# xubiker/deephisto

Hardware: AMD Instinct MI355X
Metric: 256x256 patches/sec WSI inference (predict_full_patched) (higher is better)
Workload: dtype bf16

## Files before the change

### deephisto_amd/_lib.py

```python
from __future__ import annotations

import ctypes as C
from pathlib import Path

import torch

LIB_PATH = Path(__file__).resolve().parent / "libdeephisto_hip.so"

DH_LAYOUT_NHWC, DH_LAYOUT_NCHW = 0, 1
DH_DTYPE_F32, DH_DTYPE_BF16 = 0, 1

_i32, _i64, _u32 = C.c_int32, C.c_int64, C.c_uint32
BUCKET_CB = C.CFUNCTYPE(None, C.c_int32, C.c_int64, C.c_int64, C.c_void_p)
_p = C.c_void_p

SIGNATURES = {
    "dh_abi_version": (C.c_int, []),
    "dh_last_error": (C.c_char_p, []),
    "dh_tile_grid_count": (C.c_int, [_i64, _i64, _i32, _i32, _i32, C.POINTER(_i64), C.POINTER(_i64)]),
    "dh_tile_grid": (C.c_int, [_i64, _i64, _i32, _i32, _i32, _p, _i64]),
    "dh_synth_slide": (C.c_int, [_p, _i64, _i64, _u32, _p]),
    "dh_tile_gather": (C.c_int, [_p, _i64, _i64, _p, _p, _i64, _i32, _i32, _i32, _p, _p]),
    "dh_tile_gather_aug": (C.c_int, [_p, _i64, _i64, _p, _i64, _i32, _i32, _i32, _i32, _i32, _p, _p]),
    "dh_tile_gather_raw": (C.c_int, [_p, _i64, _i64, _p, _i64, _i32, _p, _p]),
# ... 24 lines not shown
    "dh_resnet18_bucket": (C.c_int, [_p, _i32, C.POINTER(_i64), C.POINTER(_i64)]),
    "dh_train2_create": (C.c_int, [C.POINTER(_p), C.c_char_p, _i32]),
    "dh_train2_destroy": (None, [_p]),
    "dh_train2_tensor": (C.c_int, [_p, C.c_char_p, _i32, _p, _i64, _i32, _p]),
    "dh_train2_flat": (C.c_int, [_p, _i32, C.POINTER(_p), C.POINTER(_i64)]),
    "dh_train2_set_buckets": (C.c_int, [_p, _i64, _p, _p, C.POINTER(_i32)]),
    "dh_train2_bucket": (C.c_int, [_p, _i32, C.POINTER(_i64), C.POINTER(_i64)]),
    "dh_train2_forward": (C.c_int, [_p, _p, _i64, _i32, _p, _i32, _p]),
    "dh_train2_backward": (C.c_int, [_p, _p, _p]),
    "dh_train2_adam_step": (C.c_int, [_p, C.c_float, C.c_float, C.c_float, C.c_float, _i64, _p]),
    "dh_grad_pack_bf16": (C.c_int, [_p, _p, _i64, _p]),
    "dh_grad_unpack_bf16": (C.c_int, [_p, _p, _i64, C.c_float, _p]),
    "dh_train2_backward_adam": (C.c_int, [_p, _p, C.c_float, C.c_float, C.c_float, C.c_float, _i64, _p]),
    "dh_profile_start": (C.c_int, [_i32, _i32]),
    "dh_profile_stop": (C.c_int, [C.POINTER(C.c_double), C.POINTER(C.c_double), C.POINTER(_i64)]),
}


DEBUG_SIGNATURES = {
    "dh_train2_debug_act": (C.c_int, [_p, C.c_char_p, _i32, _p, _i64, _p]),
    "dh_debug_gemm1x1_bf16": (C.c_int, [_p, _p, _p, _p, _i64] + [_i32] * 8 + [_p]),
    "dh_debug_gemm1x1_fused_bf16": (C.c_int, [_p] * 7 + [_i64] + [_i32] * 8 + [_p]),
    "dh_debug_gemm1x1_bwdsums_bf16": (C.c_int, [_p] * 10 + [_i32, _p, _i64, _i32, _i32, _p]),
    "dh_debug_bn2_bf16": (C.c_int, [_p, _p, _p, _p, _i32, _p, _p, _p, _p, _i32, _p, _p, _p, _p, _i64, _i32, _p]),
    "dh_debug_stem_wgrad_bf16": (C.c_int, [_p, _p, _p, _i32, _i32, _p]),
    "dh_debug_bn2_pool_bf16": (C.c_int, [_p, _p, _p, _p, _p, _p, _p, _p, _p, _p, _p, _i32, _i32, _i32, _i32, _p]),
    "dh_debug_maxpool2_bf16": (C.c_int, [_p, _p, _p, _p, _i32, _i32, _i32, _i32, _p]),
    "dh_debug_upsample2_add_bf16": (C.c_int, [_p, _p] + [_i32] * 6 + [_p]),
    "dh_debug_avgpool_fc_dgrad2": (C.c_int, [_p, _p, _p] + [_i32] * 4 + [_p]),
    "dh_debug_wgrad_bf16": (C.c_int, [_p, _p, _p] + [_i32] * 8 + [_p]),
    "dh_debug_conv_bn_act": (C.c_int, [_p, _p, _p, _p, _p, _p] + [_i32] * 9 + [_p]),
    "dh_debug_stem_out": (C.c_int, [_p, _i64, _i32, _p, _p]),
    "dh_debug_stem_pool_bf16": (C.c_int, [_p, _p, _i64, _i64, _p, _i64, _i32, _p, _p]),
    "dh_debug_wgrad_f32": (C.c_int, [_p, _p, _p] + [_i32] * 8 + [_p]),
    "dh_debug_stem_wgrad_f32": (C.c_int, [_p, _p, _p, _i32, _i32, _p]),
    "dh_debug_dgrad_f32": (C.c_int, [_p, _p, _p, _p] + [_i32] * 7 + [_p]),
    "dh_debug_pack_f32": (C.c_int, [_p, _i32, _i32, _p, _p, _p, _p, _p]),
    "dh_debug_pack_bf16": (C.c_int, [_p, _i32, _i32, _p, _p, _p, _p, _p]),
    "dh_debug_bn_f32": (C.c_int, [_p, _p, _p, _p, _i32, _p, _p, _p, _p, _p, _p, _p, _i64, _i32, _p]),
    "dh_debug_maxpool_f32": (C.c_int, [_p, _p, _p, _p, _i32, _i32, _i32, _i32, _p]),
    "dh_debug_bn_pool_f32": (C.c_int, [_p, _p, _p, _p, _p, _p, _p, _p, _p, _i32, _i32, _i32, _i32, _p]),
    "dh_debug_stamps": (C.c_int, [_i32, _p]),
    "dh_debug_env_knobs": (C.c_int, [C.c_char_p, _i64]),
}


class DeephistoHipError(RuntimeError):
    pass


_lib = None


def lib() -> C.CDLL:
    global _lib
    if _lib is None:
        if not LIB_PATH.exists():
            raise DeephistoHipError(
                f"{LIB_PATH} is missing: build it with `python -m deephisto_amd.build` "
                "(hipcc --offload-arch=gfx950). There is no CPU fallback for the HIP path.")
        h = C.CDLL(str(LIB_PATH))
        for name, (res, args) in {**SIGNATURES, **DEBUG_SIGNATURES}.items():
            fn = getattr(h, name)
            fn.restype, fn.argtypes = res, args
        _lib = h
    return _lib
# ... 7 lines not shown
```

### deephisto_amd/csrc/resnet_kernels.hip

```cpp
#include <math.h>
#include <stdlib.h>
#include <string.h>

#include <algorithm>
#include <array>
#include <map>
#include <mutex>
#include <set>
#include <string>
#include <vector>

#include "dh_common.h"
#include "conv3_tables_host.h"

typedef float f32x16 __attribute__((ext_vector_type(16)));
typedef __bf16 bf16x8 __attribute__((ext_vector_type(8)));

namespace {

constexpr int CHUNK_BYTES = 64;
constexpr int PIX_PITCH = 80;
constexpr int FRAG_BYTES = 1024;
constexpr int SLAB_TAP = 4 * FRAG_BYTES;

// ... 532 lines not shown
            }
}

void pack_stem_weights(const float* w, int esz, std::vector<uint8_t>& out) {
  auto slot = [&](int co, int kh, int i) -> float {
    if (i < 1 || i > 21) return 0.f;
    const int kw = (i - 1) / 3, c = (i - 1) % 3;
    return w[((size_t)(co * 3 + c) * 7 + kh) * 7 + kw];
  };
  if (esz == 2) {
    out.assign((size_t)7 * 2 * 2 * FRAG_BYTES, 0);
    size_t o = 0;
    for (int kh = 0; kh < 7; ++kh)
      for (int t = 0; t < 2; ++t)
        for (int mt = 0; mt < 2; ++mt)
          for (int l = 0; l < 64; ++l)
            for (int j = 0; j < 8; ++j) {
              const uint16_t hb = host_bf16(slot(mt * 32 + (l & 31), kh, 16 * t + 8 * (l >> 5) + j));
              memcpy(&out[o], &hb, 2); o += 2;
            }
  } else {
    out.assign((size_t)7 * 11 * 2 * 256, 0);
    size_t o = 0;
    for (int kh = 0; kh < 7; ++kh)
      for (int s = 0; s < 11; ++s)
        for (int mt = 0; mt < 2; ++mt)
          for (int l = 0; l < 64; ++l) {
            const float v = slot(mt * 32 + (l & 31), kh, 2 * s + (l >> 5));
            memcpy(&out[o], &v, 4); o += 4;
          }
  }
}

void pack_stem_pool_weights(const float* w, std::vector<uint8_t>& out) {
  out.assign((size_t)SP_WBYTES, 0);
  size_t o = 0;
  for (int ks = 0; ks < SP_KS; ++ks)
    for (int mt = 0; mt < 2; ++mt)
      for (int l = 0; l < 64; ++l)
        for (int j = 0; j < 8; ++j) {
          int kh, sl;
          sp_kslot(ks, l >> 5, j, &kh, &sl);
          float v = 0.f;
          if (kh >= 0 && sl >= 1 && sl <= 21) {
            const int co = mt * 32 + (l & 31), kw = (sl - 1) / 3, c = (sl - 1) % 3;
            v = w[((size_t)(co * 3 + c) * 7 + kh) * 7 + kw];
          }
          const uint16_t hb = host_bf16(v);
          memcpy(&out[o], &hb, 2); o += 2;
        }
}

bool g_stamps_on = false;
unsigned long long* g_stamps_dev = nullptr;

struct Profiler {
  bool on = false;
  int every = 1, counter = 0;
  std::vector<hipEvent_t> ev;
  size_t used = 0;
  double flops = 0.0;
} g_prof;

std::mutex g_host_mu;
inline int current_device() { int d = 0; (void)hipGetDevice(&d); return d; }

int ensure_dyn_lds(const void* fn, int bytes) {
  static std::set<std::pair<const void*, int>> done;
  const std::pair<const void*, int> key(fn, current_device());
  std::lock_guard<std::mutex> lk(g_host_mu);
  if (done.count(key)) return DH_OK;
  DH_HIP(hipFuncSetAttribute(fn, hipFuncAttributeMaxDynamicSharedMemorySize, bytes));
  done.insert(key);
  return DH_OK;
}

template <typename T, int KS, int STRIDE, bool HALO>
int launch_conv(const ConvParams& p, hipStream_t st) {
  const int npx_lds = HALO ? p.IMGS * (p.TH + 2) * (p.TW + 2) : 256;
  const size_t lds = (size_t)KS * KS * SLAB_TAP + (size_t)npx_lds * PIX_PITCH;
  const int blocks_per_img = p.tiles_y * p.tiles_x;
  const int groups = ((p.B + p.IMGS - 1) / p.IMGS) * blocks_per_img;
  const int grid = groups * (p.Cout / 64);
// ... 517 lines not shown
  if (net->fc_w_dev) (void)hipFree(net->fc_w_dev);
  if (net->fc_b_dev) (void)hipFree(net->fc_b_dev);
  if (net->ws) (void)hipFree(net->ws);
  delete net;
}

extern "C" int dh_resnet18_set_param(dh_resnet18* net, const char* name, const float* data,
                                     int64_t n_elem) {
  DH_REQUIRE(net && name && data, "resnet18 set_param: null argument");
  const int64_t want = expected_elems(net, name);
  DH_REQUIRE(want >= 0, "resnet18 set_param: unknown parameter '%s'", name);
  DH_REQUIRE(want == n_elem, "resnet18 set_param: '%s' has %lld elements, expected %lld", name,
             (long long)n_elem, (long long)want);
  net->params[name].assign(data, data + n_elem);
  net->finalized = false;
  return DH_OK;
}

extern "C" int dh_resnet18_finalize(dh_resnet18* net, void* stream) {
  DH_REQUIRE(net != nullptr, "resnet18 finalize: null handle");
  (void)stream;
  auto get = [&](const std::string& k) -> const std::vector<float>* {
    auto it = net->params.find(k);
    return it == net->params.end() ? nullptr : &it->second;
  };
  const int esz = net->esz();
  for (size_t i = 0; i < net->convs.size(); ++i) {
    ConvLayer& c = net->convs[i];
    const auto* w = get(c.name + ".weight");
    const auto *g = get(c.bn + ".weight"), *b = get(c.bn + ".bias"), *m = get(c.bn + ".running_mean"),
               *v = get(c.bn + ".running_var");
    DH_REQUIRE(w && g && b && m && v, "resnet18 finalize: parameters of '%s' / '%s' are not all set",
               c.name.c_str(), c.bn.c_str());
    std::vector<uint8_t> packed;
    if (i == 0 && esz == 2) pack_stem_pool_weights(w->data(), packed);
    else if (i == 0) pack_stem_weights(w->data(), esz, packed);
    else pack_conv_weights(w->data(), c.cout, c.cin, c.ks, esz, packed);
    int rc = upload(packed, &c.w_dev);
    if (rc) return rc;
    const bool wide3 = esz == 2 && c.ks == 3 && c.stride == 2 && c.cout % 128 == 0 && c.cin % 16 == 0;
    const bool wide1 = esz == 2 && c.ks == 1 && c.stride == 2 && c.cout % 128 == 0 && c.cin % 16 == 0;
    if (wide3 || wide1) {
      std::vector<uint8_t> packed2;
      pack_conv_weights_wide(w->data(), c.cout, c.cin, c.ks, packed2);
      if ((rc = upload(packed2, &c.w2_dev))) return rc;
    }
    std::vector<float> sc(c.cout), sh(c.cout);
    for (int k = 0; k < c.cout; ++k) {
      const double s = (double)(*g)[k] / sqrt((double)(*v)[k] + 1e-5);
      sc[k] = (float)s;
      sh[k] = (float)((double)(*b)[k] - (double)(*m)[k] * s);
    }
    rc = upload(sc, reinterpret_cast<void**>(&c.scale_dev));
    if (rc) return rc;
    rc = upload(sh, reinterpret_cast<void**>(&c.shift_dev));
    if (rc) return rc;
  }
  const auto *fw = get("fc.weight"), *fb = get("fc.bias");
  DH_REQUIRE(fw && fb, "resnet18 finalize: fc.weight / fc.bias are not set");
  int rc = upload(*fw, reinterpret_cast<void**>(&net->fc_w_dev));
  if (rc) return rc;
  rc = upload(*fb, reinterpret_cast<void**>(&net->fc_b_dev));
  if (rc) return rc;
  net->finalized = true;
  return DH_OK;
}

static int check_forward_args(dh_resnet18* net, int64_t n, int32_t P, const void* logits) {
  DH_REQUIRE(net && (logits || n == 0), "resnet18 forward: null argument");
  DH_REQUIRE(net->finalized, "resnet18 forward: call dh_resnet18_finalize after setting parameters");
  DH_REQUIRE(n >= 0 && n <= 4096, "resnet18 forward: batch %lld out of range [0, 4096]", (long long)n);
  DH_REQUIRE(P >= 32 && P <= 1024, "resnet18 forward: patch %d out of range [32, 1024]", P);
  return DH_OK;
}

extern "C" int dh_resnet18_forward(dh_resnet18* net, const float* x, int64_t n, int32_t P,
                                   float* logits, void* stream) {
  int rc = check_forward_args(net, n, P, logits);
  if (rc) return rc;
  if (n == 0) return DH_OK;
  DH_REQUIRE(x != nullptr, "resnet18 forward: null input");
  hipStream_t st = dh::as_stream(stream);
  return net->dtype == DH_DTYPE_F32
             ? forward_impl<float>(net, x, nullptr, 0, 0, nullptr, n, P, logits, st)
// ... 68 lines not shown
  DH_LAUNCH_CHECK();
  return DH_OK;
}

namespace {
__global__ void blocked_to_nhwc_f32_kernel(const __bf16* in, float* out, int64_t n, int hw) {
  const int64_t total = n * hw * 64;
  for (int64_t i = blockIdx.x * (int64_t)blockDim.x + threadIdx.x; i < total; i += (int64_t)gridDim.x * blockDim.x) {
    const int c = (int)(i % 64);
    const int64_t px = (i / 64) % hw, b = i / 64 / hw;
    out[i] = (float)in[((b * 2 + c / 32) * hw + px) * 32 + c % 32];
  }
}
}

extern "C" int dh_debug_stem_pool_bf16(dh_resnet18* net, const uint8_t* slide_dev, int64_t slide_h, int64_t slide_w,
                                       const int32_t* yx_dev, int64_t n, int32_t P, float* out_dev, void* stream) {
  DH_REQUIRE(net && net->finalized && net->dtype == DH_DTYPE_BF16, "debug stem pool: needs a finalized bf16 network");
  DH_REQUIRE(slide_dev && yx_dev && out_dev && n > 0 && n <= (1 << 20) && P >= 32 && P <= 1024, "debug stem pool: bad arguments");
  hipStream_t st = dh::as_stream(stream);
  const int H1 = (P + 6 - 7) / 2 + 1, H2 = (H1 + 2 - 3) / 2 + 1;
  void* tmp = nullptr;
  DH_HIP(hipMalloc(&tmp, (size_t)n * H2 * H2 * 64 * 2));
  int rc = launch_stem_pool(net, nullptr, slide_dev, slide_h, slide_w, yx_dev, (int)n, P, tmp, st);
  if (!rc) {
    hipLaunchKernelGGL(blocked_to_nhwc_f32_kernel, dim3(1024), dim3(256), 0, st, static_cast<const __bf16*>(tmp), out_dev, n, H2 * H2);
    if (hipGetLastError() != hipSuccess) rc = DH_EHIP;
    (void)hipStreamSynchronize(st);
  }
  (void)hipFree(tmp);
  return rc;
}

extern "C" int dh_profile_start(int32_t sample_every, int32_t max_samples) {
  DH_REQUIRE(sample_every > 0 && max_samples > 0 && max_samples <= (1 << 20), "profile start: bad arguments");
  for (hipEvent_t e : g_prof.ev) (void)hipEventDestroy(e);
  g_prof.ev.assign((size_t)max_samples * 2, nullptr);
  for (auto& e : g_prof.ev) DH_HIP(hipEventCreate(&e));
  g_prof.every = sample_every; g_prof.counter = 0; g_prof.used = 0; g_prof.flops = 0.0;
  g_prof.on = true;
  return DH_OK;
}

extern "C" int dh_profile_stop(double* total_ms, double* total_flops, int64_t* n_samples) {
  g_prof.on = false;
  double ms = 0.0;
  for (size_t i = 0; i + 1 < g_prof.used; i += 2) {
    DH_HIP(hipEventSynchronize(g_prof.ev[i + 1]));
    float t = 0.f;
    DH_HIP(hipEventElapsedTime(&t, g_prof.ev[i], g_prof.ev[i + 1]));
    ms += t;
  }
  if (total_ms) *total_ms = ms;
  if (total_flops) *total_flops = g_prof.flops;
  if (n_samples) *n_samples = (int64_t)(g_prof.used / 2);
  for (hipEvent_t e : g_prof.ev) (void)hipEventDestroy(e);
  g_prof.ev.clear(); g_prof.used = 0;
  return DH_OK;
}

extern "C" int dh_debug_stamps(int32_t enable, unsigned long long* out64_host) {
  g_stamps_on = enable != 0;
  if (out64_host) {
    if (!g_stamps_dev) { memset(out64_host, 0, 64 * sizeof(unsigned long long)); return DH_OK; }
    DH_HIP(hipDeviceSynchronize());
    DH_HIP(hipMemcpy(out64_host, g_stamps_dev, 64 * sizeof(unsigned long long), hipMemcpyDeviceToHost));
// ... 13 lines not shown
```

### deephisto_amd/csrc/stem_pool.inc

```
#ifndef SP_ABL
#define SP_ABL 0
#endif
constexpr int SP_W = 4;
constexpr int SP_T = SP_W * 64;
constexpr int SP_CR = 2 * SP_W, SP_CC = 32;
constexpr int SP_PR = SP_W, SP_PC = 15;
constexpr int SP_WR = 2 * SP_CR + 5;
constexpr int SP_WE = 224;
#ifndef SP_PF
#define SP_PF 3
#endif
constexpr int SP_KS = 11;
constexpr int SP_WBYTES = SP_KS * 2 * FRAG_BYTES;
constexpr int SP_WINB = ((SP_WR * SP_WE * 2 + 255) / 256) * 256;
constexpr int SP_XCH = 4096;
constexpr int SP_LDS = SP_WBYTES + SP_WINB + (SP_W + 1) * SP_XCH + 512;
constexpr int SP_DW = 52;
constexpr int SP_NLOAD = (SP_WR * SP_DW + SP_T - 1) / SP_T;
static_assert(3 * ((SP_LDS + 511) / 512 * 512) <= 160 * 1024, "three workgroups per CU");

inline void sp_kslot(int ks, int hh, int j, int* kh, int* s) {
  *kh = -1; *s = 0;
  if (ks < 9) {
    const int pz = ks / 3, u = ks % 3;
    if (u == 0) { *kh = 2 * pz; *s = 8 * hh + j; }
    else if (u == 1) { *kh = 2 * pz + hh; *s = hh ? j : 16 + j; }
    else { *kh = 2 * pz + 1; *s = 8 + 8 * hh + j; }
  } else if (ks == 9) { *kh = 6; *s = 8 * hh + j; }
  else if (hh == 0) { *kh = 6; *s = 16 + j; }
}

struct StemPoolParams {
  const float* x_nchw; const uint8_t* slide; const int32_t* yx; int64_t row_bytes, slide_bytes;
  const void* w; const float* scale; const float* shift; void* out;
  int B, P, Hc, Wc, Hp, Wp, tiles_y, tiles_x, nstrips, iters;
  unsigned long long* stamps;
};

typedef unsigned short sp_u16x2 __attribute__((ext_vector_type(2)));

template <bool SRC_U8, bool STAMP>
__global__ __launch_bounds__(SP_T, 3) void stem_pool_kernel(const StemPoolParams p) {
  extern __shared__ __attribute__((aligned(16))) char smem[];
  char* w_lds = smem;
  char* win_lds = smem + SP_WBYTES;
  char* xch_lds = win_lds + SP_WINB;
  float* ss_lds = reinterpret_cast<float*>(xch_lds + (SP_W + 1) * SP_XCH);
  const int tid = threadIdx.x, lane = tid & 63, tx = lane & 31, h = lane >> 5;
  const int wave = __builtin_amdgcn_readfirstlane(tid >> 6);
  for (int i = wave; i < SP_WBYTES / 1024; i += SP_W)
    lds_dma<16>(static_cast<const char*>(p.w) + i * 1024 + lane * 16, __builtin_amdgcn_readfirstlane(lds_addr_of(w_lds + i * 1024)));
  if (tid < 128) ss_lds[tid] = tid < 64 ? p.scale[tid] : p.shift[tid - 64];
  for (int i = tid * 16; i < SP_WINB; i += SP_T * 16) *reinterpret_cast<uint4*>(win_lds + i) = make_uint4(0, 0, 0, 0);

  struct Tile { int valid, b, py0, px0, ty0, tx0, first; };
  int cur_sid = (int)blockIdx.x, cur_ty = 0, cur_b = cur_sid / p.tiles_x, cur_px0 = (cur_sid % p.tiles_x) * SP_PC, cur_it = 0;
  auto next_tile = [&]() __attribute__((always_inline)) {
    Tile t;
    t.valid = cur_sid < p.nstrips && cur_it < p.iters;
    t.b = cur_b; t.py0 = cur_ty * SP_PR; t.px0 = cur_px0; t.first = cur_ty == 0;
    t.ty0 = 0; t.tx0 = 0;
    if constexpr (SRC_U8) {
      if (t.valid) { t.ty0 = p.yx[2 * t.b]; t.tx0 = p.yx[2 * t.b + 1]; }
    }
// ... 94 lines not shown
    }
  };

  Tile cur = next_tile();
  Tile nxt = next_tile();
  Tile nn = next_tile();
#ifdef SP_STAGGER
  {
    const int ph = (int)(blockIdx.x / 256u) % 3;
    for (int i = 0; i < ph * SP_STAGGER; ++i) __builtin_amdgcn_s_sleep(32);
  }
#endif
  asm volatile("s_waitcnt vmcnt(0)" ::: "memory");
  __syncthreads();
  if (cur.valid) { load_window(cur, wr); store_window(cur, wr); }
  if (nxt.valid) load_window(nxt, wr);
  __syncthreads();

  unsigned long long tacc[6] = {0, 0, 0, 0, 0, 0};
  unsigned long long tprev = STAMP ? __builtin_readcyclecounter() : 0ull;
  auto stamp = [&](int slot) __attribute__((always_inline)) {
    if constexpr (STAMP) {
      __builtin_amdgcn_sched_barrier(0);
      const unsigned long long now = __builtin_readcyclecounter();
      __builtin_amdgcn_sched_barrier(0);
      tacc[slot] += now - tprev;
      tprev = now;
    }
  };
  typedef short sp_i16x2 __attribute__((ext_vector_type(2)));
  auto max16 = [](uint32_t a, uint32_t b) __attribute__((always_inline)) {
    return __builtin_bit_cast(uint32_t, __builtin_elementwise_max(__builtin_bit_cast(sp_i16x2, a), __builtin_bit_cast(sp_i16x2, b)));
  };
  auto hmax3 = [&](uint32_t v0) __attribute__((always_inline)) {
    const uint32_t v1 = (uint32_t)__builtin_amdgcn_update_dpp(0, (int)v0, 0x130, 0xF, 0xF, true);
    const uint32_t v2 = (uint32_t)__builtin_amdgcn_update_dpp(0, (int)v1, 0x130, 0xF, 0xF, true);
    return max16(max16(v0, v1), v2);
  };
  const int xlane = lane * 64, xsw = (lane >> 2) & 3;
  const bool even = !(tx & 1);
  const char* a_base = w_lds + lane * 16;
  const int b_base = ((4 * wave) * SP_WE + 6 * tx) * 2;
  int b_off[3];
  b_off[0] = 16 * h;
  b_off[1] = h ? SP_WE * 2 : 32;
  b_off[2] = h ? 16 : 32;
  struct SpStep { int row, shift, sel, ka, kb; };
  constexpr SpStep SCHED[14] = {
      {0, 0, 0, 0, -1}, {0, 0, 1, 1, -1}, {1, 16, 0, 2, -1},
      {2, 0, 0, 3, 0},  {2, 0, 1, 4, 1},  {3, 16, 0, 5, 2},
      {4, 0, 0, 6, 3},  {4, 0, 1, 7, 4},  {5, 16, 0, 8, 5},
      {6, 0, 0, 9, 6},  {6, 0, 1, 10, 7}, {7, 16, 0, -1, 8},
      {8, 0, 0, -1, 9}, {8, 0, 2, -1, 10}};
  auto read_a = [&](int ks, int mt) __attribute__((always_inline)) {
    return (SP_ABL & 32) ? make_uint4(lane, tid, lane, lane) : *reinterpret_cast<const uint4*>(a_base + (ks * 2 + mt) * FRAG_BYTES);
  };
  auto read_b = [&](int f) __attribute__((always_inline)) {
    const uint32_t* src = reinterpret_cast<const uint32_t*>(win_lds + b_base + b_off[SCHED[f].sel] + SCHED[f].row * SP_WE * 2 + SCHED[f].shift);
    return (SP_ABL & 32) ? make_uint4(tid, tid, lane, tid) : make_uint4(src[0], src[1], src[2], src[3]);
  };
  const f32x16 zero16 = {0.f, 0.f, 0.f, 0.f, 0.f, 0.f, 0.f, 0.f, 0.f, 0.f, 0.f, 0.f, 0.f, 0.f, 0.f, 0.f};
  auto step = [&](int it, uint32_t (&wnow)[SP_NLOAD], uint32_t (&wfly)[SP_NLOAD]) __attribute__((always_inline)) {
    if (nn.valid) load_window(nn, wfly);
    const Tile n3 = next_tile();
    stamp(0);
    uint32_t vm[2][4][2];
    if (cur.valid) {
      f32x16 acc[2][2];
      uint4 wa[SP_KS][2];
      uint4 bq[SP_PF + 1];
      auto fetch = [&](int f) __attribute__((always_inline)) {
        bq[f % (SP_PF + 1)] = read_b(f);
        if (SCHED[f].ka >= 0) { wa[SCHED[f].ka][0] = read_a(SCHED[f].ka, 0); wa[SCHED[f].ka][1] = read_a(SCHED[f].ka, 1); }
      };
#pragma unroll
      for (int f = 0; f < SP_PF; ++f) fetch(f);
#pragma unroll
      for (int f = 0; f < 14; ++f) {
        if (f + SP_PF < 14) fetch(f + SP_PF);
#pragma unroll
        for (int nt = 0; nt < 2; ++nt) {
          const int ks = nt == 0 ? SCHED[f].ka : SCHED[f].kb;
          if (ks < 0) continue;
#pragma unroll
          for (int mt = 0; mt < 2; ++mt) {
            if constexpr (SP_ABL & 1) {
              if (ks == 0) acc[mt][nt] = zero16;
              asm volatile("" :: "v"(wa[ks][mt].x), "v"(wa[ks][mt].y), "v"(wa[ks][mt].z), "v"(wa[ks][mt].w), "v"(bq[f % (SP_PF + 1)].x), "v"(bq[f % (SP_PF + 1)].y), "v"(bq[f % (SP_PF + 1)].z), "v"(bq[f % (SP_PF + 1)].w));
            } else {
              acc[mt][nt] = __builtin_amdgcn_mfma_f32_32x32x16_bf16(__builtin_bit_cast(bf16x8, wa[ks][mt]), __builtin_bit_cast(bf16x8, bq[f % (SP_PF + 1)]),
                                                                    ks == 0 ? zero16 : acc[mt][nt], 0, 0, 0);
            }
          }
        }
      }
      stamp(1);
      const int r0 = 2 * cur.py0, c0 = 2 * cur.px0 - 1;
      const bool interior = r0 + SP_CR <= p.Hc && c0 >= 0 && c0 + SP_CC <= p.Wc;
      char* slot = xch_lds + (wave < SP_W - 1 ? wave : SP_W - 1 + (it & 1)) * SP_XCH + xlane;
      auto bn_pack = [&](auto inside) __attribute__((always_inline)) {
        constexpr bool INSIDE = decltype(inside)::value;
        uint32_t okm[2] = {~0u, ~0u};
        if constexpr (!INSIDE) {
          const bool col_ok = (c0 + tx) >= 0 && (c0 + tx) < p.Wc;
          okm[0] = col_ok && (r0 + 2 * wave) < p.Hc ? ~0u : 0u;
          okm[1] = col_ok && (r0 + 2 * wave + 1) < p.Hc ? ~0u : 0u;
        }
        typedef float f32x2_t __attribute__((ext_vector_type(2)));
        typedef __bf16 bf16x2_t __attribute__((ext_vector_type(2)));
#pragma unroll
        for (int mt = 0; mt < 2; ++mt)
#pragma unroll
          for (int pr = 0; pr < 2; ++pr) {
            uint32_t rb[2][2];
#pragma unroll
            for (int gg = 0; gg < 2; ++gg) {
              const int g = 2 * pr + gg;
              const float4 sc = *reinterpret_cast<const float4*>(ss_lds + (mt * 4 + g) * 8 + 4 * h);
              const float4 sh = *reinterpret_cast<const float4*>(ss_lds + 64 + (mt * 4 + g) * 8 + 4 * h);
              uint32_t row[2][2];
#pragma unroll
              for (int nt = 0; nt < 2; ++nt) {
                const f32x2_t lo = __builtin_elementwise_fma(f32x2_t{acc[mt][nt][4 * g + 0], acc[mt][nt][4 * g + 1]}, f32x2_t{sc.x, sc.y}, f32x2_t{sh.x, sh.y});
                const f32x2_t hi = __builtin_elementwise_fma(f32x2_t{acc[mt][nt][4 * g + 2], acc[mt][nt][4 * g + 3]}, f32x2_t{sc.z, sc.w}, f32x2_t{sh.z, sh.w});
                row[nt][0] = __builtin_bit_cast(uint32_t, __builtin_convertvector(lo, bf16x2_t));
                row[nt][1] = __builtin_bit_cast(uint32_t, __builtin_convertvector(hi, bf16x2_t));
                if constexpr (!INSIDE) { row[nt][0] &= okm[nt]; row[nt][1] &= okm[nt]; }
              }
              rb[gg][0] = row[1][0]; rb[gg][1] = row[1][1];
              vm[mt][g][0] = max16(row[0][0], row[1][0]);
              vm[mt][g][1] = max16(row[0][1], row[1][1]);
            }
            *reinterpret_cast<uint4*>(slot + (((mt * 2 + pr) ^ xsw) << 4)) = make_uint4(rb[0][0], rb[0][1], rb[1][0], rb[1][1]);
          }
      };
      if (interior) bn_pack(std::true_type{});
      else bn_pack(std::false_type{});
      stamp(2);
    }
    asm volatile("s_waitcnt lgkmcnt(0)" ::: "memory");
    __builtin_amdgcn_s_barrier();
    asm volatile("" ::: "memory");
    stamp(5);
    if (nxt.valid) store_window(nxt, wnow);
    stamp(4);
    if (cur.valid) {
      const char* prev = xch_lds + (wave > 0 ? wave - 1 : SP_W - 1 + ((it + 1) & 1)) * SP_XCH + xlane;
      const bool have_prev = wave > 0 || !cur.first;
      const int py = cur.py0 + wave, px = cur.px0 + (tx >> 1);
      const bool st_ok = even && (tx >> 1) < SP_PC && py < p.Hp && px < p.Wp;
      const int plane = p.Hp * p.Wp * 32;
      __bf16* out = static_cast<__bf16*>(p.out) + (int64_t)cur.b * 2 * plane + (py * p.Wp + px) * 32;
      uint4 pvq[4];
#pragma unroll
      for (int q = 0; q < 4; ++q) pvq[q] = make_uint4(0u, 0u, 0u, 0u);
      if (have_prev) {
#pragma unroll
        for (int q = 0; q < 4; ++q) pvq[q] = *reinterpret_cast<const uint4*>(prev + ((q ^ xsw) << 4));
      }
#pragma unroll
      for (int mt = 0; mt < 2; ++mt)
#pragma unroll
        for (int pr = 0; pr < 2; ++pr) {
          const uint4 pv = pvq[mt * 2 + pr];
          uint32_t v[4] = {max16(vm[mt][2 * pr][0], pv.x), max16(vm[mt][2 * pr][1], pv.y),
                           max16(vm[mt][2 * pr + 1][0], pv.z), max16(vm[mt][2 * pr + 1][1], pv.w)};
          if constexpr (!(SP_ABL & 8)) {
#pragma unroll
            for (int i = 0; i < 4; ++i) v[i] = max16(hmax3(v[i]), 0u);
          }
          uint32_t a0 = v[0], a1 = v[1], b0 = v[2], b1 = v[3];
          { const auto r = __builtin_amdgcn_permlane32_swap(a0, b0, false, false); a0 = r[0]; b0 = r[1]; }
          { const auto r = __builtin_amdgcn_permlane32_swap(a1, b1, false, false); a1 = r[0]; b1 = r[1]; }
          if constexpr (SP_ABL & 16) asm volatile("" :: "v"(a0), "v"(a1), "v"(b0), "v"(b1));
          else if (st_ok) *reinterpret_cast<uint4*>(out + mt * plane + (2 * pr + h) * 8) = make_uint4(a0, a1, b0, b1);
        }
      stamp(3);
    }
    asm volatile("s_waitcnt lgkmcnt(0)" ::: "memory");
    __builtin_amdgcn_s_barrier();
    asm volatile("" ::: "memory");
    stamp(5);
    cur = nxt;
    nxt = nn;
    nn = n3;
  };
  for (int it = 0; it < p.iters; it += 2) {
    step(it, wr, wr2);
    step(it + 1, wr2, wr);
  }
  if constexpr (STAMP) {
    if (tid == 0 && p.stamps) {
      for (int i = 0; i < 6; ++i) atomicAdd(p.stamps + i, tacc[i]);
      atomicAdd(p.stamps + 6, 1ull);
    }
  }
}
```

### include/deephisto_hip_debug.h

```cpp
#ifndef DEEPHISTO_HIP_DEBUG_H
#define DEEPHISTO_HIP_DEBUG_H

#include "deephisto_hip.h"

#ifdef __cplusplus
extern "C" {
#endif

int dh_train2_debug_act(dh_train2* net, const char* conv_name, int32_t what, float* out_dev, int64_t n_elem, void* stream);

int dh_debug_pack_bf16(const float* w_dev, int32_t cout, int32_t cin, uint16_t* wf_tile, uint16_t* wd_tile, uint16_t* wf_elem,
                       uint16_t* wd_elem, void* stream);
int dh_debug_gemm1x1_bf16(const uint16_t* a_dev, const uint16_t* w_dev, const uint16_t* res_dev, uint16_t* out_dev, int64_t M,
                          int32_t N, int32_t K, int32_t stride, int32_t Ho, int32_t Wo, int32_t Hi, int32_t Wi, int32_t repeat,
                          void* stream);
int dh_debug_gemm1x1_fused_bf16(const uint16_t* a_dev, const uint16_t* w_dev, const uint16_t* res_dev, const uint16_t* mask_dev,
                                uint16_t* out_dev, float* mean_dev, float* invstd_dev, int64_t M, int32_t N, int32_t K, int32_t stride,
                                int32_t Ho, int32_t Wo, int32_t Hi, int32_t Wi, int32_t repeat, void* stream);
int dh_debug_gemm1x1_bwdsums_bf16(const uint16_t* a_dev, const uint16_t* w_dev, const uint16_t* res_dev, const uint16_t* mask_dev,
                                  uint16_t* out_dev, const uint16_t* z_dev, const float* mean_dev, const float* invstd_dev,
                                  const float* scale_dev, const float* shift_dev, int32_t relu_mode, float* sums_dev, int64_t M, int32_t N,
                                  int32_t K, void* stream);
int dh_debug_bn2_bf16(const uint16_t* z_dev, const uint16_t* res_dev, const float* gamma_dev, const float* beta_dev, int32_t relu,
                      uint16_t* y_dev, float* mean_dev, float* invstd_dev, const uint16_t* dy_dev, int32_t relu_mode, uint16_t* dz_dev,
                      uint16_t* g_out_dev, float* dgamma_dev, float* dbeta_dev, int64_t rows, int32_t C, void* stream);
int dh_debug_bn2_pool_bf16(const uint16_t* z_dev, const float* gamma_dev, const float* beta_dev, uint16_t* pooled_dev, uint8_t* idx_dev,
                           float* mean_dev, float* invstd_dev, const uint16_t* dpool_dev, uint16_t* dz_dev, float* dgamma_dev,
                           float* dbeta_dev, int32_t B, int32_t Hi, int32_t Wi, int32_t C, void* stream);
int dh_debug_maxpool2_bf16(const uint16_t* x_dev, uint16_t* y_dev, const uint16_t* dy_dev, uint16_t* dx_dev, int32_t B, int32_t Hi,
                           int32_t Wi, int32_t C, void* stream);
int dh_debug_upsample2_add_bf16(const uint16_t* t_dev, uint16_t* dx_dev, int32_t B, int32_t Ho, int32_t Wo, int32_t Hi, int32_t Wi,
                                int32_t C, void* stream);
int dh_debug_avgpool_fc_dgrad2(const float* dlogits_dev, const float* w_dev, uint16_t* dx_dev, int32_t B, int32_t HW, int32_t C,
                               int32_t n_cls, void* stream);
int dh_debug_stem_wgrad_bf16(const uint16_t* dz_dev, const float* x_nchw_dev, float* dw_dev, int32_t B, int32_t P, void* stream);
int dh_debug_wgrad_bf16(const uint16_t* dz_dev, const uint16_t* x_dev, float* dw_dev, int32_t B, int32_t Hi, int32_t Wi,
                        int32_t cin, int32_t cout, int32_t ks, int32_t stride, int32_t repeat, void* stream);

int dh_debug_conv_bn_act(const void* in_dev, const float* w_host, const float* scale_host,
                         const float* shift_host, const void* res_dev, void* out_dev, int32_t B,
                         int32_t H, int32_t W, int32_t cin, int32_t cout, int32_t ks, int32_t stride,
                         int32_t relu, int32_t dtype, void* stream);
int dh_debug_stem_out(dh_resnet18* net, int64_t n, int32_t patch, float* out_dev, void* stream);
int dh_debug_stem_pool_bf16(dh_resnet18* net, const uint8_t* slide_dev, int64_t slide_h, int64_t slide_w, const int32_t* yx_dev,
                            int64_t n, int32_t patch, float* out_dev, void* stream);
int dh_debug_wgrad_f32(const float* dz_dev, const float* x_dev, float* dw_dev, int32_t B, int32_t Hi, int32_t Wi,
                       int32_t cin, int32_t cout, int32_t ks, int32_t stride, int32_t mode, void* stream);
int dh_debug_stem_wgrad_f32(const float* dz_dev, const float* x_nchw_dev, float* dw_dev, int32_t B, int32_t P, void* stream);
int dh_debug_dgrad_f32(const float* dz_dev, const float* w_dev, const float* res_dev, float* dx_dev, int32_t B, int32_t Hi,
                       int32_t Wi, int32_t cin, int32_t cout, int32_t ks, int32_t stride, void* stream);
int dh_debug_pack_f32(const float* w_dev, int32_t cout, int32_t cin, float* wf_tile, float* wd_tile, float* wf_elem, float* wd_elem,
                      void* stream);
int dh_debug_bn_f32(const float* z_dev, const float* gamma_dev, const float* beta_dev, const float* res_dev, int32_t relu,
                    float* y_dev, const float* dy_dev, float* dz_dev, float* g_dev, float* dgamma_dev, float* dbeta_dev,
                    float* stats_out_dev, int64_t rows, int32_t C, void* stream);
int dh_debug_maxpool_f32(const float* x_dev, float* y_dev, const float* dy_dev, float* dx_dev, int32_t B, int32_t Hi, int32_t Wi,
                         int32_t C, void* stream);
int dh_debug_bn_pool_f32(const float* z_dev, const float* gamma_dev, const float* beta_dev, float* pooled_dev, uint8_t* idx_dev,
                         const float* dpool_dev, float* dz_dev, float* dgamma_dev, float* dbeta_dev, int32_t B, int32_t Hi, int32_t Wi,
                         int32_t C, void* stream);
int dh_debug_stamps(int32_t enable, unsigned long long* out64_host);
int dh_debug_env_knobs(char* buf_host, int64_t cap);

#ifdef __cplusplus
}
#endif
#endif
```

Baseline: 219,900.

## Max-pool raw stem conv outputs before BN by folding BN sign into weights

Folds the sign of each channel's BN scale into the packed stem weights so the scale becomes non-negative. With a positive scale, the affine BN commutes with max, so the 3x3 max-pool can run on the raw f32 MFMA accumulators first and BN is applied only to the pooled values. The MFMA operands are swapped so the horizontal pool is done within a lane's registers, with a permlane32 swap for the edge column, instead of DPP cross-lane maxes. Results go through an LDS transpose for coalesced bf16 stores. This cuts per-element BN FMAs and conversions but doubles the exchange data (f32 instead of bf16) and adds an extra LDS round trip.

```diff
diff --git a/deephisto_amd/_lib.py b/deephisto_amd/_lib.py
--- a/deephisto_amd/_lib.py
+++ b/deephisto_amd/_lib.py
@@ -80,6 +80,7 @@
     "dh_debug_conv_bn_act": (C.c_int, [_p, _p, _p, _p, _p, _p] + [_i32] * 9 + [_p]),
     "dh_debug_stem_out": (C.c_int, [_p, _i64, _i32, _p, _p]),
     "dh_debug_stem_pool_bf16": (C.c_int, [_p, _p, _i64, _i64, _p, _i64, _i32, _p, _p]),
+    "dh_debug_pack_stem_pool": (C.c_int, [_p, _p, _p, _p]),
     "dh_debug_wgrad_f32": (C.c_int, [_p, _p, _p] + [_i32] * 8 + [_p]),
     "dh_debug_stem_wgrad_f32": (C.c_int, [_p, _p, _p, _i32, _i32, _p]),
     "dh_debug_dgrad_f32": (C.c_int, [_p, _p, _p, _p] + [_i32] * 7 + [_p]),
diff --git a/deephisto_amd/csrc/resnet_kernels.hip b/deephisto_amd/csrc/resnet_kernels.hip
--- a/deephisto_amd/csrc/resnet_kernels.hip
+++ b/deephisto_amd/csrc/resnet_kernels.hip
@@ -588,7 +588,7 @@
   }
 }
 
-void pack_stem_pool_weights(const float* w, std::vector<uint8_t>& out) {
+void pack_stem_pool_weights(const float* w, std::vector<float>& scale, std::vector<uint8_t>& out) {
   out.assign((size_t)SP_WBYTES, 0);
   size_t o = 0;
   for (int ks = 0; ks < SP_KS; ++ks)
@@ -601,10 +601,12 @@
           if (kh >= 0 && sl >= 1 && sl <= 21) {
             const int co = mt * 32 + (l & 31), kw = (sl - 1) / 3, c = (sl - 1) % 3;
             v = w[((size_t)(co * 3 + c) * 7 + kh) * 7 + kw];
+            if (scale[co] < 0.f) v = -v;
           }
           const uint16_t hb = host_bf16(v);
           memcpy(&out[o], &hb, 2); o += 2;
         }
+  for (float& s : scale) s = fabsf(s);
 }
 
 bool g_stamps_on = false;
@@ -1188,8 +1190,14 @@
                *v = get(c.bn + ".running_var");
     DH_REQUIRE(w && g && b && m && v, "resnet18 finalize: parameters of '%s' / '%s' are not all set",
                c.name.c_str(), c.bn.c_str());
+    std::vector<float> sc(c.cout), sh(c.cout);
+    for (int k = 0; k < c.cout; ++k) {
+      const double s = (double)(*g)[k] / sqrt((double)(*v)[k] + 1e-5);
+      sc[k] = (float)s;
+      sh[k] = (float)((double)(*b)[k] - (double)(*m)[k] * s);
+    }
     std::vector<uint8_t> packed;
-    if (i == 0 && esz == 2) pack_stem_pool_weights(w->data(), packed);
+    if (i == 0 && esz == 2) pack_stem_pool_weights(w->data(), sc, packed);
     else if (i == 0) pack_stem_weights(w->data(), esz, packed);
     else pack_conv_weights(w->data(), c.cout, c.cin, c.ks, esz, packed);
     int rc = upload(packed, &c.w_dev);
@@ -1200,12 +1208,6 @@
       std::vector<uint8_t> packed2;
       pack_conv_weights_wide(w->data(), c.cout, c.cin, c.ks, packed2);
       if ((rc = upload(packed2, &c.w2_dev))) return rc;
-    }
-    std::vector<float> sc(c.cout), sh(c.cout);
-    for (int k = 0; k < c.cout; ++k) {
-      const double s = (double)(*g)[k] / sqrt((double)(*v)[k] + 1e-5);
-      sc[k] = (float)s;
-      sh[k] = (float)((double)(*b)[k] - (double)(*m)[k] * s);
     }
     rc = upload(sc, reinterpret_cast<void**>(&c.scale_dev));
     if (rc) return rc;
@@ -1340,6 +1342,16 @@
   return rc;
 }
 
+extern "C" int dh_debug_pack_stem_pool(const float* w_host, const float* scale_host, uint16_t* packed_out, float* scale_out) {
+  DH_REQUIRE(w_host && scale_host && packed_out && scale_out, "debug pack stem pool: null argument");
+  std::vector<float> sc(scale_host, scale_host + 64);
+  std::vector<uint8_t> packed;
+  pack_stem_pool_weights(w_host, sc, packed);
+  memcpy(packed_out, packed.data(), packed.size());
+  memcpy(scale_out, sc.data(), sc.size() * sizeof(float));
+  return DH_OK;
+}
+
 extern "C" int dh_profile_start(int32_t sample_every, int32_t max_samples) {
   DH_REQUIRE(sample_every > 0 && max_samples > 0 && max_samples <= (1 << 20), "profile start: bad arguments");
   for (hipEvent_t e : g_prof.ev) (void)hipEventDestroy(e);
diff --git a/deephisto_amd/csrc/stem_pool.inc b/deephisto_amd/csrc/stem_pool.inc
--- a/deephisto_amd/csrc/stem_pool.inc
+++ b/deephisto_amd/csrc/stem_pool.inc
@@ -30,6 +30,8 @@
   else if (hh == 0) { *kh = 6; *s = 16 + j; }
 }
 
+constexpr int sp_col(int m) { return 16 * ((m >> 2) & 1) + 4 * (m >> 3) + (m & 3); }
+
 struct StemPoolParams {
   const float* x_nchw; const uint8_t* slide; const int32_t* yx; int64_t row_bytes, slide_bytes;
   const void* w; const float* scale; const float* shift; void* out;
@@ -190,15 +192,9 @@
   auto max16 = [](uint32_t a, uint32_t b) __attribute__((always_inline)) {
     return __builtin_bit_cast(uint32_t, __builtin_elementwise_max(__builtin_bit_cast(sp_i16x2, a), __builtin_bit_cast(sp_i16x2, b)));
   };
-  auto hmax3 = [&](uint32_t v0) __attribute__((always_inline)) {
-    const uint32_t v1 = (uint32_t)__builtin_amdgcn_update_dpp(0, (int)v0, 0x130, 0xF, 0xF, true);
-    const uint32_t v2 = (uint32_t)__builtin_amdgcn_update_dpp(0, (int)v1, 0x130, 0xF, 0xF, true);
-    return max16(max16(v0, v1), v2);
-  };
   const int xlane = lane * 64, xsw = (lane >> 2) & 3;
-  const bool even = !(tx & 1);
   const char* a_base = w_lds + lane * 16;
-  const int b_base = ((4 * wave) * SP_WE + 6 * tx) * 2;
+  const int b_base = ((4 * wave) * SP_WE + 6 * sp_col(tx)) * 2;
   int b_off[3];
   b_off[0] = 16 * h;
   b_off[1] = h ? SP_WE * 2 : 32;
@@ -222,7 +218,7 @@
     if (nn.valid) load_window(nn, wfly);
     const Tile n3 = next_tile();
     stamp(0);
-    uint32_t vm[2][4][2];
+    float hab[2][8];
     if (cur.valid) {
       f32x16 acc[2][2];
       uint4 wa[SP_KS][2];
@@ -246,7 +242,7 @@
               if (ks == 0) acc[mt][nt] = zero16;
               asm volatile("" :: "v"(wa[ks][mt].x), "v"(wa[ks][mt].y), "v"(wa[ks][mt].z), "v"(wa[ks][mt].w), "v"(bq[f % (SP_PF + 1)].x), "v"(bq[f % (SP_PF + 1)].y), "v"(bq[f % (SP_PF + 1)].z), "v"(bq[f % (SP_PF + 1)].w));
             } else {
-              acc[mt][nt] = __builtin_amdgcn_mfma_f32_32x32x16_bf16(__builtin_bit_cast(bf16x8, wa[ks][mt]), __builtin_bit_cast(bf16x8, bq[f % (SP_PF + 1)]),
+              acc[mt][nt] = __builtin_amdgcn_mfma_f32_32x32x16_bf16(__builtin_bit_cast(bf16x8, bq[f % (SP_PF + 1)]), __builtin_bit_cast(bf16x8, wa[ks][mt]),
                                                                     ks == 0 ? zero16 : acc[mt][nt], 0, 0, 0);
             }
           }
@@ -254,46 +250,51 @@
       }
       stamp(1);
       const int r0 = 2 * cur.py0, c0 = 2 * cur.px0 - 1;
-      const bool interior = r0 + SP_CR <= p.Hc && c0 >= 0 && c0 + SP_CC <= p.Wc;
+      const float ninf = -__builtin_inff();
+      if (c0 < 0) {
+#pragma unroll
+        for (int mt = 0; mt < 2; ++mt)
+#pragma unroll
+          for (int nt = 0; nt < 2; ++nt) acc[mt][nt][0] = h ? acc[mt][nt][0] : ninf;
+      }
+      if (((p.Wc & 1) && c0 + SP_CC > p.Wc) || ((p.Hc & 1) && r0 + SP_CR > p.Hc)) {
+#pragma unroll
+        for (int nt = 0; nt < 2; ++nt) {
+          const int wc = r0 + 2 * wave + nt < p.Hc ? p.Wc - c0 - 16 * h : 0;
+#pragma unroll
+          for (int mt = 0; mt < 2; ++mt)
+#pragma unroll
+            for (int k = 0; k < 16; ++k) acc[mt][nt][k] = k < wc ? acc[mt][nt][k] : ninf;
+        }
+      }
+      auto hpool = [&](const f32x16& r, float (&o)[8]) __attribute__((always_inline)) {
+        if constexpr (SP_ABL & (8 | 128)) {
+#pragma unroll
+          for (int k = 0; k < 8; ++k) o[k] = r[2 * k];
+        } else {
+#pragma unroll
+          for (int k = 0; k < 7; ++k) o[k] = __builtin_elementwise_maximum(__builtin_elementwise_maximum(r[2 * k], r[2 * k + 1]), r[2 * k + 2]);
+          const auto sw = __builtin_amdgcn_permlane32_swap(__builtin_bit_cast(uint32_t, r[0]), __builtin_bit_cast(uint32_t, r[1]), false, false);
+          o[7] = __builtin_elementwise_maximum(__builtin_elementwise_maximum(r[14], r[15]), __builtin_bit_cast(float, (uint32_t)sw[1]));
+        }
+      };
+      float hb[2][8];
+#pragma unroll
+      for (int mt = 0; mt < 2; ++mt) {
+        float ha[8];
+        hpool(acc[mt][0], ha);
+        hpool(acc[mt][1], hb[mt]);
+#pragma unroll
+        for (int k = 0; k < 8; ++k) {
+          if constexpr (SP_ABL & (8 | 128)) { hab[mt][k] = ha[k]; asm volatile("" :: "v"(hb[mt][k])); }
+          else hab[mt][k] = __builtin_elementwise_maximum(ha[k], hb[mt][k]);
+        }
+      }
       char* slot = xch_lds + (wave < SP_W - 1 ? wave : SP_W - 1 + (it & 1)) * SP_XCH + xlane;
-      auto bn_pack = [&](auto inside) __attribute__((always_inline)) {
-        constexpr bool INSIDE = decltype(inside)::value;
-        uint32_t okm[2] = {~0u, ~0u};
-        if constexpr (!INSIDE) {
-          const bool col_ok = (c0 + tx) >= 0 && (c0 + tx) < p.Wc;
-          okm[0] = col_ok && (r0 + 2 * wave) < p.Hc ? ~0u : 0u;
-          okm[1] = col_ok && (r0 + 2 * wave + 1) < p.Hc ? ~0u : 0u;
-        }
-        typedef float f32x2_t __attribute__((ext_vector_type(2)));
-        typedef __bf16 bf16x2_t __attribute__((ext_vector_type(2)));
-#pragma unroll
-        for (int mt = 0; mt < 2; ++mt)
-#pragma unroll
-          for (int pr = 0; pr < 2; ++pr) {
-            uint32_t rb[2][2];
-#pragma unroll
-            for (int gg = 0; gg < 2; ++gg) {
-              const int g = 2 * pr + gg;
-              const float4 sc = *reinterpret_cast<const float4*>(ss_lds + (mt * 4 + g) * 8 + 4 * h);
-              const float4 sh = *reinterpret_cast<const float4*>(ss_lds + 64 + (mt * 4 + g) * 8 + 4 * h);
-              uint32_t row[2][2];
-#pragma unroll
-              for (int nt = 0; nt < 2; ++nt) {
-                const f32x2_t lo = __builtin_elementwise_fma(f32x2_t{acc[mt][nt][4 * g + 0], acc[mt][nt][4 * g + 1]}, f32x2_t{sc.x, sc.y}, f32x2_t{sh.x, sh.y});
-                const f32x2_t hi = __builtin_elementwise_fma(f32x2_t{acc[mt][nt][4 * g + 2], acc[mt][nt][4 * g + 3]}, f32x2_t{sc.z, sc.w}, f32x2_t{sh.z, sh.w});
-                row[nt][0] = __builtin_bit_cast(uint32_t, __builtin_convertvector(lo, bf16x2_t));
-                row[nt][1] = __builtin_bit_cast(uint32_t, __builtin_convertvector(hi, bf16x2_t));
-                if constexpr (!INSIDE) { row[nt][0] &= okm[nt]; row[nt][1] &= okm[nt]; }
-              }
-              rb[gg][0] = row[1][0]; rb[gg][1] = row[1][1];
-              vm[mt][g][0] = max16(row[0][0], row[1][0]);
-              vm[mt][g][1] = max16(row[0][1], row[1][1]);
-            }
-            *reinterpret_cast<uint4*>(slot + (((mt * 2 + pr) ^ xsw) << 4)) = make_uint4(rb[0][0], rb[0][1], rb[1][0], rb[1][1]);
-          }
-      };
-      if (interior) bn_pack(std::true_type{});
-      else bn_pack(std::false_type{});
+#pragma unroll
+      for (int q = 0; q < 4; ++q)
+        *reinterpret_cast<float4*>(slot + ((q ^ xsw) << 4)) = make_float4(hb[q >> 1][4 * (q & 1)], hb[q >> 1][4 * (q & 1) + 1],
+                                                                         hb[q >> 1][4 * (q & 1) + 2], hb[q >> 1][4 * (q & 1) + 3]);
       stamp(2);
     }
     asm volatile("s_waitcnt lgkmcnt(0)" ::: "memory");
@@ -303,36 +304,69 @@
     if (nxt.valid) store_window(nxt, wnow);
     stamp(4);
     if (cur.valid) {
-      const char* prev = xch_lds + (wave > 0 ? wave - 1 : SP_W - 1 + ((it + 1) & 1)) * SP_XCH + xlane;
+      int xs = wave > 0 ? wave - 1 : SP_W - 1 + ((it + 1) & 1);
+      asm volatile("" : "+s"(xs));
+      const char* prev = xch_lds + xs * SP_XCH + xlane;
       const bool have_prev = wave > 0 || !cur.first;
-      const int py = cur.py0 + wave, px = cur.px0 + (tx >> 1);
-      const bool st_ok = even && (tx >> 1) < SP_PC && py < p.Hp && px < p.Wp;
+      float v[2][8];
+      if (have_prev) {
+        float4 pv[4];
+#pragma unroll
+        for (int q = 0; q < 4; ++q) pv[q] = *reinterpret_cast<const float4*>(prev + ((q ^ xsw) << 4));
+#pragma unroll
+        for (int mt = 0; mt < 2; ++mt)
+#pragma unroll
+          for (int k = 0; k < 8; ++k) {
+            const float4 q4 = pv[mt * 2 + (k >> 2)];
+            const float pk = (k & 3) == 0 ? q4.x : (k & 3) == 1 ? q4.y : (k & 3) == 2 ? q4.z : q4.w;
+            if constexpr (SP_ABL & (8 | 128)) { v[mt][k] = hab[mt][k]; asm volatile("" :: "v"(pk)); }
+            else v[mt][k] = __builtin_elementwise_maximum(hab[mt][k], pk);
+          }
+      } else {
+#pragma unroll
+        for (int mt = 0; mt < 2; ++mt)
+#pragma unroll
+          for (int k = 0; k < 8; ++k) v[mt][k] = hab[mt][k];
+      }
+      char* tb = xch_lds + xs * SP_XCH;
+      int ln = lane;
+      asm volatile("" : "+v"(ln));
+      const int ltx = ln & 31, lh = ln >> 5;
+      const float bn_s[2] = {ss_lds[tx], ss_lds[32 + tx]}, bn_t[2] = {ss_lds[64 + tx], ss_lds[96 + tx]};
+      asm volatile("s_waitcnt lgkmcnt(0)" ::: "memory");
+#pragma unroll
+      for (int mt = 0; mt < 2; ++mt)
+#pragma unroll
+        for (int k = 0; k < 8; ++k) {
+          const float y = (SP_ABL & 128) ? v[mt][k] : __builtin_fmaf(bn_s[mt], v[mt][k], bn_t[mt]);
+          *reinterpret_cast<float*>(tb + (8 * lh + k) * 256 + mt * 128 + ((ltx ^ (k & 2 ? 4 : 0)) << 2)) = y;
+        }
+      asm volatile("s_waitcnt lgkmcnt(0)" ::: "memory");
+      const int py = cur.py0 + wave, o = ln & 7;
       const int plane = p.Hp * p.Wp * 32;
-      __bf16* out = static_cast<__bf16*>(p.out) + (int64_t)cur.b * 2 * plane + (py * p.Wp + px) * 32;
-      uint4 pvq[4];
-#pragma unroll
-      for (int q = 0; q < 4; ++q) pvq[q] = make_uint4(0u, 0u, 0u, 0u);
-      if (have_prev) {
-#pragma unroll
-        for (int q = 0; q < 4; ++q) pvq[q] = *reinterpret_cast<const uint4*>(prev + ((q ^ xsw) << 4));
-      }
-#pragma unroll
-      for (int mt = 0; mt < 2; ++mt)
-#pragma unroll
-        for (int pr = 0; pr < 2; ++pr) {
-          const uint4 pv = pvq[mt * 2 + pr];
-          uint32_t v[4] = {max16(vm[mt][2 * pr][0], pv.x), max16(vm[mt][2 * pr][1], pv.y),
-                           max16(vm[mt][2 * pr + 1][0], pv.z), max16(vm[mt][2 * pr + 1][1], pv.w)};
-          if constexpr (!(SP_ABL & 8)) {
-#pragma unroll
-            for (int i = 0; i < 4; ++i) v[i] = max16(hmax3(v[i]), 0u);
-          }
-          uint32_t a0 = v[0], a1 = v[1], b0 = v[2], b1 = v[3];
-          { const auto r = __builtin_amdgcn_permlane32_swap(a0, b0, false, false); a0 = r[0]; b0 = r[1]; }
-          { const auto r = __builtin_amdgcn_permlane32_swap(a1, b1, false, false); a1 = r[0]; b1 = r[1]; }
-          if constexpr (SP_ABL & 16) asm volatile("" :: "v"(a0), "v"(a1), "v"(b0), "v"(b1));
-          else if (st_ok) *reinterpret_cast<uint4*>(out + mt * plane + (2 * pr + h) * 8) = make_uint4(a0, a1, b0, b1);
-        }
+      __bf16* out = static_cast<__bf16*>(p.out) + (int64_t)cur.b * 2 * plane + (o >> 2) * plane + (py * p.Wp + cur.px0) * 32 + (o & 3) * 8;
+      typedef float f32x2_t __attribute__((ext_vector_type(2)));
+      typedef __bf16 bf16x2_t __attribute__((ext_vector_type(2)));
+#pragma unroll
+      for (int u = 0; u < 2; ++u) {
+        const int pp = (ln >> 3) + 8 * u;
+        const char* src = tb + pp * 256 + o * 32;
+        const int sw = (pp & 2) << 3;
+        const float4 f0 = *reinterpret_cast<const float4*>(src + sw), f1 = *reinterpret_cast<const float4*>(src + (sw ^ 16));
+        uint32_t d[4];
+        if constexpr (SP_ABL & 128) {
+          d[0] = __builtin_bit_cast(uint32_t, f0.x); d[1] = __builtin_bit_cast(uint32_t, f0.z);
+          d[2] = __builtin_bit_cast(uint32_t, f1.x); d[3] = __builtin_bit_cast(uint32_t, f1.z);
+          asm volatile("" :: "v"(f0.y), "v"(f0.w), "v"(f1.y), "v"(f1.w));
+        } else {
+          d[0] = max16(__builtin_bit_cast(uint32_t, __builtin_convertvector((f32x2_t{f0.x, f0.y}), bf16x2_t)), 0u);
+          d[1] = max16(__builtin_bit_cast(uint32_t, __builtin_convertvector((f32x2_t{f0.z, f0.w}), bf16x2_t)), 0u);
+          d[2] = max16(__builtin_bit_cast(uint32_t, __builtin_convertvector((f32x2_t{f1.x, f1.y}), bf16x2_t)), 0u);
+          d[3] = max16(__builtin_bit_cast(uint32_t, __builtin_convertvector((f32x2_t{f1.z, f1.w}), bf16x2_t)), 0u);
+        }
+        if constexpr (SP_ABL & 16) asm volatile("" :: "v"(d[0]), "v"(d[1]), "v"(d[2]), "v"(d[3]));
+        else if (pp < SP_PC && py < p.Hp && cur.px0 + pp < p.Wp) *reinterpret_cast<uint4*>(out + pp * 32) = make_uint4(d[0], d[1], d[2], d[3]);
+      }
       stamp(3);
     }
     asm volatile("s_waitcnt lgkmcnt(0)" ::: "memory");
diff --git a/include/deephisto_hip_debug.h b/include/deephisto_hip_debug.h
--- a/include/deephisto_hip_debug.h
+++ b/include/deephisto_hip_debug.h
@@ -44,6 +44,7 @@
 int dh_debug_stem_out(dh_resnet18* net, int64_t n, int32_t patch, float* out_dev, void* stream);
 int dh_debug_stem_pool_bf16(dh_resnet18* net, const uint8_t* slide_dev, int64_t slide_h, int64_t slide_w, const int32_t* yx_dev,
                             int64_t n, int32_t patch, float* out_dev, void* stream);
+int dh_debug_pack_stem_pool(const float* w_host, const float* scale_host, uint16_t* packed_out, float* scale_out);
 int dh_debug_wgrad_f32(const float* dz_dev, const float* x_dev, float* dw_dev, int32_t B, int32_t Hi, int32_t Wi,
                        int32_t cin, int32_t cout, int32_t ks, int32_t stride, int32_t mode, void* stream);
 int dh_debug_stem_wgrad_f32(const float* dz_dev, const float* x_nchw_dev, float* dw_dev, int32_t B, int32_t P, void* stream);
```

Result: no change. 221,700 (median of 6 runs) (+0.8%).
